# omkhairate/MetalPathtracer

Hardware: AMD Instinct MI355X
Metric: Mrays/s at 1920x1080x256spp on scene.xml (higher is better)
Workload: dtype f32; 1 GPU; scene.xml 1920x1080 x 256 spp per step, depth 8 (181 steps timed); prims=4971, bvh_nodes=2289, bvh_builder=device, rng=philox4x32-10 (pixel,sample,bounce), pipeline=wave-local wavefront, reference-order walk, parallelism=8x8-tile interleave over 1 rank(s), rays=161154900585

## Files before the change

metalpathtracer_amd/csrc/mpt_device.h:

```cpp
#pragma once
#include <hip/hip_runtime.h>
#include <stdint.h>

#include "mpt_lean_entry.h"
#include "mpt_lean_tiles.h"
#include "mpt_lds_cfg.h"

#define MPT_WAVE 64
#define MPT_NSHARD 16
#define MPT_NGROUP 8
#define MPT_NONE 0xFFFFFFFFu

struct F3 {
    float x, y, z;
};
__device__ __forceinline__ F3 f3(float x, float y, float z) { return F3{x, y, z}; }
__device__ __forceinline__ F3 operator+(F3 a, F3 b) { return F3{a.x + b.x, a.y + b.y, a.z + b.z}; }
__device__ __forceinline__ F3 operator-(F3 a, F3 b) { return F3{a.x - b.x, a.y - b.y, a.z - b.z}; }
__device__ __forceinline__ F3 operator*(F3 a, float s) { return F3{a.x * s, a.y * s, a.z * s}; }
__device__ __forceinline__ F3 operator*(float s, F3 a) { return F3{s * a.x, s * a.y, s * a.z}; }
__device__ __forceinline__ F3 operator-(F3 a) { return F3{-a.x, -a.y, -a.z}; }
__device__ __forceinline__ float dot3(F3 a, F3 b) { return a.x * b.x + a.y * b.y + a.z * b.z; }
__device__ __forceinline__ F3 cross3(F3 a, F3 b) {
    return F3{a.y * b.z - a.z * b.y, a.z * b.x - a.x * b.z, a.x * b.y - a.y * b.x};
// ... 139 lines not shown
typedef const __attribute__((address_space(3))) uint32_t* LdsWords;

struct SceneDev {
    const float4* nodes;
    const float4* prims;
    const float4* mats;
    uint32_t n_nodes;
    uint32_t n_lds_nodes;
    uint32_t n_lds_prims;
    uint32_t n_lds_mats;
    uint32_t n_prims;
    uint32_t n_mats;
    uint32_t lds_prim_off;
    uint32_t lds_mat_off;
};
__device__ __forceinline__ int prim_type(float4 p0) { return __float_as_int(p0.w) & 1; }
__device__ __forceinline__ uint32_t prim_ref_leaf(float4 p0) { return (uint32_t)__float_as_int(p0.w) >> 1; }

#ifdef MPT_CLOCK_STAMP
__device__ unsigned long long g_clock[2];
#define MPT_CLOCK_BEGIN() const unsigned long long clk_t0_ = __builtin_amdgcn_s_memtime(), clk_r0_ = __builtin_amdgcn_s_memrealtime()
#define MPT_CLOCK_END()                                                                    \
    do {                                                                                   \
        if ((threadIdx.x & 63u) == 0) {                                                    \
            atomicAdd(&g_clock[0], __builtin_amdgcn_s_memtime() - clk_t0_);                \
            atomicAdd(&g_clock[1], __builtin_amdgcn_s_memrealtime() - clk_r0_);            \
        }                                                                                  \
    } while (0)
#else
#define MPT_CLOCK_BEGIN() do { } while (0)
#define MPT_CLOCK_END() do { } while (0)
#endif

__device__ __forceinline__ bool first_active_lane() {
    const uint32_t me = __builtin_amdgcn_mbcnt_hi(~0u, __builtin_amdgcn_mbcnt_lo(~0u, 0u));
    return me == (uint32_t)__builtin_amdgcn_readfirstlane((int)me);
}

__device__ __forceinline__ uint32_t wave_max_u32(uint32_t v) {
#pragma unroll
    for (int off = 32; off > 0; off >>= 1) {
        const uint32_t other = (uint32_t)__shfl_xor((int)v, off);
        v = other > v ? other : v;
    }
    return v;
}

struct WorkCount {
    uint32_t node_visits, aabb_hits, prim_tests;
    uint32_t node_iters, prim_iters, outer_iters;
#ifdef MPT_DEBUG_WAVE_TIMES
    unsigned long long t_box, t_leaf;
    uint32_t wait_leaf, wait_done;
#endif
#ifdef MPT_OT_TIMES
    unsigned long long ot_node_cycles, ot_leaf_cycles, ot_node_trips, ot_leaf_trips, ot_rounds;
    unsigned long long ot_node_lanes, ot_leaf_lanes;
    unsigned long long ot_lds_nodes, ot_glb_nodes, ot_lds_prims, ot_glb_prims;
    unsigned long long ot_pops, ot_pop_iters, ot_pop_calls, ot_pop_wave_iters;
#endif
};
#ifdef MPT_DEBUG_WAVE_TIMES
#define MPT_TIC(var) unsigned long long var = __builtin_amdgcn_s_memtime()
#define MPT_TOC(acc, var)                                          \
    do {                                                           \
        unsigned long long now_ = __builtin_amdgcn_s_memtime();    \
        (acc) += now_ - (var);                                     \
        (var) = now_;                                              \
    } while (0)
#else
#define MPT_TIC(var) do { } while (0)
#define MPT_TOC(acc, var) do { } while (0)
#endif
struct BoxLoopIdle {
#ifdef MPT_DEBUG_WAVE_TIMES
    uint32_t my_trips = 0, round_trips = 0;
    __device__ __forceinline__ void trip(bool searching) {
        my_trips += searching ? 1u : 0u;
        round_trips++;
    }
    template <bool COUNT>
    __device__ __forceinline__ void book(bool holds_leaf, WorkCount& wc) const {
        if (!COUNT) return;
        if (holds_leaf) wc.wait_leaf += round_trips - my_trips;
        else wc.wait_done += round_trips - my_trips;
    }
#else
    __device__ __forceinline__ void trip(bool) {}
    template <bool COUNT>
    __device__ __forceinline__ void book(bool, WorkCount&) const {}
#endif
};

struct Prim3 {
    float4 p0, p1, p2;
};
typedef const __attribute__((address_space(3))) char* LdsBytes;
__device__ __forceinline__ uint32_t mul_u24(uint32_t a, uint32_t b) { return (uint32_t)__umul24(a, b); }
__device__ __forceinline__ void sphere_cam_terms(F3 o, float4 p0, float4& p1, float4& p2) {
    const F3 oc = o - f3(p0.x, p0.y, p0.z);
    const float radius = p1.x;
    p1.z = dot3(oc, oc) - radius * radius;
    p2.x = oc.x;
    p2.y = oc.y;
    p2.z = oc.z;
}
template <bool LEAN = false, bool PRIMARY = false>
__device__ __forceinline__ Prim3 load_prim(const SceneDev& sc, LdsNodes lds, uint32_t i, F3 o = F3{0.0f, 0.0f, 0.0f}) {
    Prim3 r;
    if (LEAN) {
        const uint32_t off = mul_u24(i, 48u);
        if (i < sc.n_lds_prims) {
            const LdsNodes q = (LdsNodes)((LdsBytes)lds + (sc.lds_prim_off * 16u + off));
            const v4f a = q[0], b = q[1], c = q[2];
            r.p0 = make_float4(a.x, a.y, a.z, a.w);
            r.p1 = make_float4(b.x, b.y, b.z, b.w);
            r.p2 = make_float4(c.x, c.y, c.z, c.w);
        } else {
            const float4* q = (const float4*)((const char*)sc.prims + off);
            r.p0 = q[0];
            r.p1 = q[1];
            r.p2 = q[2];
            if (PRIMARY && prim_type(r.p0) == 0) sphere_cam_terms(o, r.p0, r.p1, r.p2);
        }
        return r;
    }
    if (i < sc.n_lds_prims) {
        const LdsNodes q = lds + sc.lds_prim_off + 3u * i;
        const v4f a = q[0], b = q[1], c = q[2];
        r.p0 = make_float4(a.x, a.y, a.z, a.w);
        r.p1 = make_float4(b.x, b.y, b.z, b.w);
        r.p2 = make_float4(c.x, c.y, c.z, c.w);
    } else {
        r.p0 = sc.prims[3 * i];
        r.p1 = sc.prims[3 * i + 1];
        r.p2 = sc.prims[3 * i + 2];
    }
    return r;
}

// ... 38 lines not shown
            const float cc = cam_terms ? p1.z : dot3(oc, oc) - radius * radius;
            const float disc = b * b - a * cc;
            if (!(b >= 0.0f) && disc > 0.0f) {
                const float sq = sqrtf(disc);
                const float temp = (-b - sq) / a;
                const bool closer = temp < best_t && temp > 0.0001f;
                best_t = closer ? temp : best_t;
                best_prim = closer ? (int)(first + k) : best_prim;
            }
        }
    }
}


#ifndef MPT_LEAF_EARLY
#define MPT_LEAF_EARLY 8u
#endif
#define MPT_NODE_HOLD 0x80000000u
__device__ __forceinline__ bool slab_hit(float4 n0, float4 n1, F3 o, float idx, float idy, float idz, float best_t) {
    float t0 = (n0.x - o.x) * idx, t1 = (n1.x - o.x) * idx;
    float lo = fmaxf(0.0001f, idx < 0.0f ? t1 : t0);
    float hi = fminf(best_t, idx < 0.0f ? t0 : t1);
    t0 = (n0.y - o.y) * idy;
    t1 = (n1.y - o.y) * idy;
    lo = fmaxf(lo, idy < 0.0f ? t1 : t0);
    hi = fminf(hi, idy < 0.0f ? t0 : t1);
    t0 = (n0.z - o.z) * idz;
    t1 = (n1.z - o.z) * idz;
    lo = fmaxf(lo, idz < 0.0f ? t1 : t0);
    hi = fminf(hi, idz < 0.0f ? t0 : t1);
    return hi > lo;
}
static_assert(MPT_LEAN_LEAF_BIT == MPT_NODE_HOLD && MPT_NODE_TAIL < MPT_NODE_HOLD, "mpt_lean_entry.h: the leaf bit and the tail marker");
template <bool COUNT, bool ALL_LDS, bool BUDGETED, bool LEAN = false, bool PRIMARY = false>
__device__ __forceinline__ bool closest_hit_resume(const SceneDev& sc, LdsNodes lds_nodes, F3 o, F3 d, uint32_t& node,
                                                   float& best_t, int& best_prim, uint32_t budget, WorkCount& wc,
                                                   uint32_t min_active = 0u, LdsNodes tail_cfg = nullptr, uint32_t tile_class = 0u) {
    constexpr bool TILES = PRIMARY && LEAN && ALL_LDS;
    const bool tile_skip = TILES && (tile_class & MPT_LEAN_TILES_SKIP) != 0u;
    float idx = 0.0f, idy = 0.0f, idz = 0.0f;
    const uint32_t n_nodes = sc.n_nodes, n_lds = sc.n_lds_nodes;
    uint32_t i = (tile_class & MPT_LEAN_TILES_MASK_BITS) != 0u ? MPT_NODE_TAIL : n_nodes;
    if (!tile_skip) {
    mpt_rcp3(d.x, d.y, d.z, idx, idy, idz);
    i = (d.x != d.x || d.y != d.y || d.z != d.z) ? n_nodes : node;
    uint32_t trips = 0;
    MPT_TIC(tic_);
    for (;;) {
        uint32_t skip = 0;
        unsigned long long search_mask = __ballot(i < n_nodes);
        const uint32_t n_entered0 = (uint32_t)__popcll(search_mask), n_entered = max(n_entered0, 1u);
        BoxLoopIdle idle;
        uint32_t n_searching = n_entered0;
        while (n_searching * MPT_LEAF_EARLY >= n_entered && (!BUDGETED || trips < budget)) {
            const bool searching = LEAN ?__builtin_amdgcn_inverse_ballot_w64(search_mask) : i < n_nodes;
            idle.trip(searching);
            const uint32_t j = LEAN ? i : (i < n_nodes - 1u ? i : n_nodes - 1u);
            float4 n0 = make_float4(0, 0, 0, 0), n1 = n0;
            bool box = false;
            if (searching) {
                if (ALL_LDS || j < n_lds) {
                    const v4f a = lds_nodes[2 * j], b = lds_nodes[2 * j + 1];
                    n0 = make_float4(a.x, a.y, a.z, a.w);
                    n1 = make_float4(b.x, b.y, b.z, b.w);
                } else {
                    n0 = sc.nodes[2 * j];
                    n1 = sc.nodes[2 * j + 1];
                }
                box = slab_hit(n0, n1, o, idx, idy, idz, best_t);
            }
            const uint32_t A = __float_as_uint(n0.w), B = __float_as_uint(n1.w);
            if (COUNT) {
                wc.node_visits += searching ? 1u : 0u;
                wc.aabb_hits += (searching && box) ? 1u : 0u;
                if (first_active_lane()) wc.node_iters++;
            }
            const uint32_t next = box ? A : B;
            i = searching ? next : i;
            skip = searching ? B : skip;
            if (BUDGETED) trips++;
            search_mask = __ballot(i < n_nodes);
            n_searching = (uint32_t)__popcll(search_mask);
        }
        idle.template book<COUNT>((i & MPT_NODE_HOLD) != 0u, wc);
        MPT_TOC(wc.t_box, tic_);
        if ((i & MPT_NODE_HOLD) != 0u) {
            const uint32_t enc = i & ~MPT_NODE_HOLD;
            if (COUNT && first_active_lane()) wc.outer_iters++;
            leaf_test<COUNT, LEAN, PRIMARY>(sc, lds_nodes, enc >> 4, (enc & 15u) + 1u, o, d, best_t, best_prim, wc);
            i = skip;
        }
        MPT_TOC(wc.t_leaf, tic_);
        if (BUDGETED && trips >= budget) break;
        const unsigned long long going = __ballot(i < n_nodes);
        if (going == 0ull) break;
        if (BUDGETED && (uint32_t)__popcll(going) < min_active) break;
    }
    }
    if (LEAN && ALL_LDS) {
        if (i == MPT_NODE_TAIL) {
            const bool d_ok = fmaxf(fmaxf(fabsf(d.x), fabsf(d.y)), fabsf(d.z)) <= MPT_LEAN_ENTRY_DMAX;
            bool hit;
            uint32_t leaf;
            if (PRIMARY) {
                const LdsWords w = (LdsWords)tail_cfg;
                leaf = w[CFG_TAIL_W_LEAF];
                hit = d_ok && w[CFG_TAIL_W_PRIMARY] != 0u;
            } else {
                const v4f tlo = tail_cfg[CFG_TAIL_LO], thi = tail_cfg[CFG_TAIL_HI];
                leaf = __float_as_uint(tlo.w);
                hit = d_ok && tlo.x <= o.x && o.x <= thi.x && tlo.y <= o.y && o.y <= thi.y && tlo.z <= o.z && o.z <= thi.z;
            }
#if !defined(MPT_LEAN_TAIL_NO_SLAB)
            if (__ballot(!hit) != 0ull) {
                if (!hit) {
                    const v4f a = tail_cfg[CFG_TAIL_N0], b = tail_cfg[CFG_TAIL_N1];
                    hit = slab_hit(make_float4(a.x, a.y, a.z, a.w), make_float4(b.x, b.y, b.z, b.w), o, idx, idy, idz, best_t);
                }
            }
#endif
            if (hit) {
                const uint32_t enc = (uint32_t)__builtin_amdgcn_readfirstlane((int)leaf) & ~MPT_NODE_HOLD;
                if (TILES) {
                    uint32_t m = tile_skip ? tile_class & MPT_LEAN_TILES_MASK_BITS : (2u << (enc & 15u)) - 1u;
                    do {
                        const uint32_t s = (uint32_t)__builtin_ctz(m), run = (uint32_t)__builtin_ctz(~(m >> s));
                        leaf_test<COUNT, LEAN, PRIMARY>(sc, lds_nodes, (enc >> 4) + s, run, o, d, best_t, best_prim, wc);
                        m &= ~(((1u << run) - 1u) << s);
                    } while (m != 0u);
                } else {
                    leaf_test<COUNT, LEAN, PRIMARY>(sc, lds_nodes, enc >> 4, (enc & 15u) + 1u, o, d, best_t, best_prim, wc);
                }
            }
        }
    }
    node = i;
    return i >= n_nodes;
}

template <bool COUNT, bool ALL_LDS>
__device__ __forceinline__ void closest_hit(const SceneDev& sc, LdsNodes lds_nodes, F3 o, F3 d,
                                            float& best_t, int& best_prim, WorkCount& wc) {
    uint32_t node = 0;
    best_t = INFINITY;
    best_prim = -1;
    closest_hit_resume<COUNT, ALL_LDS, false>(sc, lds_nodes, o, d, node, best_t, best_prim, 0xFFFFFFFFu, wc);
}

struct HitInfo {
// ... 162 lines not shown
```

metalpathtracer_amd/csrc/mpt_hip.hip:

```cpp
#include <hip/hip_runtime.h>

#include <math.h>
#include <stdint.h>
#include <stdio.h>
#include <string.h>

#include <algorithm>
#include <chrono>
#include <condition_variable>
#include <deque>
#include <mutex>
#include <thread>
#include <map>
#include <memory>
#include <exception>
#include <string>
#include <type_traits>
#include <vector>

#include "mpt.h"
#include "mpt_accel.h"
#include "mpt_scene_layout.h"
#include "mpt_env.h"
#include "mpt_device.h"
// ... 205 lines not shown
    std::unique_ptr<Submitter> sub;
    uint64_t async_jobs = 0;
    uint64_t gate_resident = 0;
    uint64_t gate_timeout = 0;
    uint64_t async_call_us_max = 0;
    hipStream_t stream = nullptr;
    Lane lane[2];
    int next_lane = 0;
    hipEvent_t last_resolved = nullptr;
    hipEvent_t last_traced = nullptr;
    int resolve_wgs_per_cu = 2;
    bool sync_render = false;
    uint32_t launch_seq = 0;
    Lane* last_trace_lane = nullptr;
    int lane_order = 5;
    Event ev_sum_op;
    hipDeviceProp_t prop;
    std::string err;
    std::mutex err_mu;
    bool have_scene = false;
    struct OtPoint {
        uint32_t threads, wgs_per_cu, lds_nodes, lds_prims;
    } ot_pt[2] = {{MPT_OT_THREADS, MPT_OT_WGS_PER_CU, 0, 0}, {MPT_OT6_THREADS, (MPT_OT6_WAVES * 256) / MPT_OT6_THREADS, 0, 0}};
    int ot_occ = 0;
    bool tile_order_forced = false;
    uint32_t ot_stack_depth = 8;
    mpt_build::ScratchPool build_pool;
    DevMem<> spare_block;
    DevMem<> in_block;
    OtBudgets ot_budgets = default_ot_budgets();
    float acc_cull_rel = 9.765625e-4f;
    mpt_uniforms u;
    bool have_uniforms = false;
    uint32_t W = 0, H = 0;
    DevMem<float4> d_accum[2];
    int cur_target = 0;
    DevMem<float4> d_sum_own;
    float4* d_sum = nullptr;
    DevMem<uint32_t> d_tile_xy;
    uint32_t tile_W = 0, tile_H = 0, tile_rank = 0, tile_nranks = 0, tile_count = 0;
    int tile_mode_built = -1;
    int tile_order_mode = 0;
    DevMem<uint32_t> d_pixel_seed;
    float seed_rs[3] = {NAN, NAN, NAN};
    uint32_t seed_W = 0, seed_H = 0;
    int wg_size = 0;
    const void* occ_fun = nullptr;
    size_t occ_lds = 0;
    int occ_per_cu = 0;
    bool time_kernels = true;
    WaveBudgets budgets = default_budgets();
    uint32_t wl_min = 0, wl_div = 32;
    bool wl_lean = true;
    bool lean_tiles = true;
    bool lean_sky_resolve = true;
    LeanCdivCache lean_cdiv;
    DevMem<uint32_t> d_cdiv_bad;
    uint32_t wl_block = MPT_WL_BLOCK;
    int wgs_per_cu = 0;
    size_t lds_budget = 78 * 1024;
    mpt_stats stats = {};
    uint64_t guide_epoch = 1;
    uint64_t tile_class_builds = 0;
    GuideState gd;
    DenoiseState dn;
    DevMem<float4> d_m2;
    AdaptiveTiles ad;
    TemporalState tp;
    SvgfState sv;
    DisplayState dp;
    AoState ao;
    LightState lights;
    DirectState di;
    RestirState rs;
    NeeState nee;
    int32_t light_sampling = MPT_LIGHT_SAMPLING_AREA;
    uint32_t light_candidates = 1u;
    int dp_px = 4;
    bool dp_hist_agg = true;
};

struct TraceKernel {
    const void* fn;
    const char* name;
    int wg_max;
};
enum { TK_PLAIN = 0, TK_CORUN = 1, TK_LEAN = 2, TK_SIX = 4 };
static const struct TraceKernelRow {
    int pipeline;
    bool count, all_lds;
    int variant;
    TraceKernel k;
} g_trace_kernels[] = {
    {MPT_PIPE_WAVEFRONT, true, true, TK_PLAIN, {(const void*)k_step<true, true>, "k_step", 1024}},
    {MPT_PIPE_WAVEFRONT, true, false, TK_PLAIN, {(const void*)k_step<true, false>, "k_step", 1024}},
    {MPT_PIPE_WAVEFRONT, false, true, TK_PLAIN, {(const void*)k_step<false, true>, "k_step", 1024}},
    {MPT_PIPE_WAVEFRONT, false, false, TK_PLAIN, {(const void*)k_step<false, false>, "k_step", 1024}},
    {MPT_PIPE_MEGAKERNEL, true, true, TK_PLAIN, {(const void*)k_megakernel<true, true>, "k_megakernel", 1024}},
    {MPT_PIPE_MEGAKERNEL, true, false, TK_PLAIN, {(const void*)k_megakernel<true, false>, "k_megakernel", 1024}},
    {MPT_PIPE_MEGAKERNEL, false, true, TK_PLAIN, {(const void*)k_megakernel<false, true>, "k_megakernel", 1024}},
    {MPT_PIPE_MEGAKERNEL, false, false, TK_PLAIN, {(const void*)k_megakernel<false, false>, "k_megakernel", 1024}},
    {MPT_PIPE_ORDERED, false, true, TK_SIX, {(const void*)k_ordered<false, true, MPT_OT6_WAVES>, "k_ordered", MPT_OT6_THREADS}},
    {MPT_PIPE_ORDERED, false, false, TK_SIX, {(const void*)k_ordered<false, false, MPT_OT6_WAVES>, "k_ordered", MPT_OT6_THREADS}},
    {MPT_PIPE_ORDERED, true, true, TK_PLAIN, {(const void*)k_ordered<true, true>, "k_ordered", MPT_OT_THREADS}},
    {MPT_PIPE_ORDERED, true, false, TK_PLAIN, {(const void*)k_ordered<true, false>, "k_ordered", MPT_OT_THREADS}},
    {MPT_PIPE_ORDERED, false, true, TK_PLAIN, {(const void*)k_ordered<false, true>, "k_ordered", MPT_OT_THREADS}},
// ... 56 lines not shown
        case MPT_ERR_INVALID_ARG: return "invalid argument";
        case MPT_ERR_NO_DEVICE: return "no HIP device";
        case MPT_ERR_HIP: return "HIP runtime error";
        case MPT_ERR_BAD_SCENE: return "malformed scene arrays";
        case MPT_ERR_NOT_READY: return "scene, uniforms or size not set";
        case MPT_ERR_OVERFLOW: return "ray queue overflow";
    }
    return "unknown status";
}
extern "C" const char* mpt_last_error(const mpt_ctx* ctx) { return ctx ? ctx->err.c_str() : "null context"; }

static int create_impl(int device_ordinal, mpt_ctx** out) {
    if (!out) return MPT_ERR_INVALID_ARG;
    *out = nullptr;
    int n = 0;
    if (hipGetDeviceCount(&n) != hipSuccess || n <= 0) return MPT_ERR_NO_DEVICE;
    if (device_ordinal < 0 || device_ordinal >= n) return MPT_ERR_NO_DEVICE;
    std::unique_ptr<mpt_ctx> ctx(new mpt_ctx());
    ctx->device = device_ordinal;
    if (hipSetDevice(device_ordinal) != hipSuccess) return MPT_ERR_HIP;
    if (hipGetDeviceProperties(&ctx->prop, device_ordinal) != hipSuccess) return MPT_ERR_HIP;
    if (const char* lo = getenv("MPT_LANE_ORDER")) ctx->lane_order = atoi(lo);
    if (const char* rw = getenv("MPT_RESOLVE_WGS")) ctx->resolve_wgs_per_cu = std::max(0, atoi(rw));
    int prio_lo = 0, prio_hi = 0;
    if (hipDeviceGetStreamPriorityRange(&prio_lo, &prio_hi) != hipSuccess) prio_lo = prio_hi = 0;
    for (Lane& L : ctx->lane) {
        const int prio = &L == &ctx->lane[0] ? prio_hi : prio_lo;
        if (((ctx->lane_order & 2) ? L.stream.create(hipStreamCreateWithPriority, hipStreamNonBlocking, prio)
                                   : L.stream.create(hipStreamCreateWithFlags, hipStreamNonBlocking)) != hipSuccess ||
            L.d_desc.alloc(sizeof(PassDesc)) != hipSuccess || hipMemset(L.d_desc.get(), 0, sizeof(PassDesc)) != hipSuccess ||
            L.d_ctr.alloc(MPT_CTR_WORDS * 4) != hipSuccess || hipMemset(L.d_ctr.get(), 0, MPT_CTR_WORDS * 4) != hipSuccess ||
            L.h_done.alloc(64, hipHostMallocMapped) != hipSuccess || L.h_desc.alloc(sizeof(PassDesc)) != hipSuccess ||
            L.ev0.create(hipEventCreate) != hipSuccess || L.ev1.create(hipEventCreate) != hipSuccess ||
            L.ev_resolved.create(hipEventCreate) != hipSuccess || L.ev_traced.create(hipEventCreateWithFlags, hipEventDisableTiming) != hipSuccess)
            return MPT_ERR_HIP;
        memset((void*)L.h_done.get(), 0, 64);
    }
    ctx->stream = ctx->lane[0].stream.get();
    if (ctx->ev_sum_op.create(hipEventCreate) != hipSuccess) return MPT_ERR_HIP;
    const char* e;
    if ((e = getenv("MPT_WG_SIZE"))) ctx->wg_size = atoi(e);
    if ((e = getenv("MPT_WGS_PER_CU"))) ctx->wgs_per_cu = atoi(e);
    if ((e = getenv("MPT_LDS_BYTES"))) ctx->lds_budget = (size_t)atol(e);
    ctx->time_kernels = !((e = getenv("MPT_NO_KERNEL_EVENTS")) && atoi(e));
    if ((e = getenv("MPT_WL_BLOCK")) && atoi(e) >= 64) ctx->wl_block = (uint32_t)atoi(e) & ~63u;
    if ((e = getenv("MPT_DISPLAY_PX")) && (atoi(e) == 1 || atoi(e) == 4)) ctx->dp_px = atoi(e);
    if ((e = getenv("MPT_DISPLAY_HIST"))) ctx->dp_hist_agg = strcmp(e, "plain") != 0;
    if ((e = getenv("MPT_BUDGETS"))) fill_budgets(e, ctx->budgets.b, MPT_WL_LEVELS - 1u);
    if ((e = getenv("MPT_MIN_ACTIVE"))) fill_min_active(e, ctx->budgets.min_active, MPT_WL_LEVELS);
    if ((e = getenv("MPT_LIGHT_BUDGET")) && atoi(e) >= 1) {
        uint32_t b = (uint32_t)atoi(e);
        for (uint32_t k = 0; k + 1 < MPT_WL_LEVELS; ++k) ctx->budgets.b[k] = b > (1u << 28) ? b : std::min<uint64_t>((uint64_t)b << k, MPT_WL_NO_BUDGET);
    }
    if ((e = getenv("MPT_WL_MIN")) && atoi(e) >= 64) ctx->wl_min = (uint32_t)atoi(e) & ~63u;
    if ((e = getenv("MPT_TILE_ORDER"))) {
        ctx->tile_order_mode = atoi(e);
        ctx->tile_order_forced = true;
    }
    if ((e = getenv("MPT_OT_OCC")) && (atoi(e) == 5 || atoi(e) == 6)) ctx->ot_occ = atoi(e);
    if ((e = getenv("MPT_WL_DIV")) && atoi(e) >= 1) ctx->wl_div = (uint32_t)atoi(e);
    if ((e = getenv("MPT_WL_LEAN"))) ctx->wl_lean = atoi(e) != 0;
    if ((e = getenv("MPT_LEAN_TILES"))) ctx->lean_tiles = atoi(e) != 0;
    if ((e = getenv("MPT_LEAN_SKY_RESOLVE"))) ctx->lean_sky_resolve = atoi(e) != 0;
    if ((e = getenv("MPT_OT_STACK")) && atoi(e) >= 2 && atoi(e) <= (int)MPT_OT_PARK) ctx->ot_stack_depth = (uint32_t)atoi(e);
    unsigned ot[MPT_OT_MLEVELS];
    if ((e = getenv("MPT_OT_BUDGETS")))
        for (unsigned k = 0, n = parse_uint_list(e, ot, MPT_OT_MLEVELS); k < n && k + 1 < MPT_OT_MLEVELS; ++k) ctx->ot_budgets.trips[k] = ot[k] < 1 ? 1 : ot[k];
    if ((e = getenv("MPT_OT_MIN_ACTIVE")))
        for (unsigned k = 0, n = parse_uint_list(e, ot, MPT_OT_MLEVELS); k < n; ++k) ctx->ot_budgets.min_active[k] = ot[k] > 64 ? 64 : ot[k];
    if ((e = getenv("MPT_OT_INPLACE")) && atoi(e) >= 1) ctx->ot_budgets.inplace_min = (uint32_t)atoi(e);
    if ((e = getenv("MPT_OT_CULL_REL")) && atof(e) > 0.0) ctx->acc_cull_rel = (float)atof(e);
    if (ctx->wg_size < 64 || ctx->wg_size > 1024 || (ctx->wg_size & 63)) ctx->wg_size = 0;
    if (ctx->lds_budget > 160 * 1024) ctx->lds_budget = 160 * 1024;
    for (const TraceKernelRow& r : g_trace_kernels) hipFuncSetAttribute(r.k.fn, hipFuncAttributeMaxDynamicSharedMemorySize, 160 * 1024);
    hipFuncSetAttribute((const void*)k_trace_rays_ordered, hipFuncAttributeMaxDynamicSharedMemorySize, 160 * 1024);
    hipFuncSetAttribute((const void*)k_trace_rays, hipFuncAttributeMaxDynamicSharedMemorySize, 160 * 1024);
    hipFuncSetAttribute((const void*)k_dn_guide, hipFuncAttributeMaxDynamicSharedMemorySize, 160 * 1024);
    for (const void* k : {(const void*)k_occluded_ref<false>, (const void*)k_occluded_ref<true>, (const void*)k_occluded_own, (const void*)k_ao<MPT_AO_REF>,
                          (const void*)k_ao<MPT_AO_REF_ALL_LDS>, (const void*)k_ao<MPT_AO_OWN>, (const void*)k_direct<MPT_AO_REF>,
                          (const void*)k_direct<MPT_AO_REF_ALL_LDS>, (const void*)k_direct<MPT_AO_OWN>, (const void*)k_nee<MPT_AO_REF>,
                          (const void*)k_nee<MPT_AO_REF_ALL_LDS>, (const void*)k_nee<MPT_AO_OWN>, (const void*)k_direct_cone<MPT_AO_REF>,
                          (const void*)k_direct_cone<MPT_AO_REF_ALL_LDS>, (const void*)k_direct_cone<MPT_AO_OWN>, (const void*)k_nee_cone<MPT_AO_REF>,
                          (const void*)k_nee_cone<MPT_AO_REF_ALL_LDS>, (const void*)k_nee_cone<MPT_AO_OWN>, (const void*)k_nee_adaptive<MPT_AO_REF>,
                          (const void*)k_nee_adaptive<MPT_AO_REF_ALL_LDS>, (const void*)k_nee_adaptive<MPT_AO_OWN>,
                          (const void*)k_nee_adaptive_cone<MPT_AO_REF>, (const void*)k_nee_adaptive_cone<MPT_AO_REF_ALL_LDS>,
                          (const void*)k_nee_adaptive_cone<MPT_AO_OWN>, (const void*)k_restir_initial<MPT_AO_REF>,
                          (const void*)k_restir_initial<MPT_AO_REF_ALL_LDS>, (const void*)k_restir_initial<MPT_AO_OWN>,
                          (const void*)k_restir_merge<MPT_AO_REF, true>, (const void*)k_restir_merge<MPT_AO_REF_ALL_LDS, true>,
                          (const void*)k_restir_merge<MPT_AO_OWN, true>, (const void*)k_restir_merge<MPT_AO_REF, false>,
                          (const void*)k_restir_merge<MPT_AO_REF_ALL_LDS, false>, (const void*)k_restir_merge<MPT_AO_OWN, false>})
        hipFuncSetAttribute(k, hipFuncAttributeMaxDynamicSharedMemorySize, 160 * 1024);
    *out = ctx.release();
    return MPT_OK;
}

extern "C" int mpt_destroy(mpt_ctx* ctx) {
    if (!ctx) return MPT_ERR_INVALID_ARG;
    stop_submit(ctx);
    hipSetDevice(ctx->device);
    for (Lane& L : ctx->lane)
        if (L.stream) hipStreamSynchronize(L.stream.get());
    delete ctx;
    return MPT_OK;
}

static void size_lds_images(mpt_ctx* ctx) {
// ... 444 lines not shown
    return slots_items;
}

static int fill_pass_params(mpt_ctx* ctx, Lane& L, const mpt_render_params* p, uint32_t sample_begin, uint32_t S, int tile_mode,
                            const TileOverride* ovr, PassParams& pp) {
    const uint32_t tiles_x = (ctx->W + 7) / 8;
    pp.scene = scene_dev(ctx);
    for (int i = 0; i < 2; ++i) pp.q[i] = QueueDev{L.q_od[i].get(), L.q_dt[i].get(), L.q_tl[i].get(), L.q_ia[i].get()};
    pp.shard_cap = L.shard_cap;
    pp.desc = L.d_desc.get();
    pp.ctr = L.d_ctr.get();
    pp.slots = L.d_slots.get();
    pp.pixel_seed = ctx->d_pixel_seed.get();
    const mpt_uniforms& u = ctx->u;
    pp.cam = F3{u.cameraPosition[0], u.cameraPosition[1], u.cameraPosition[2]};
    pp.first = F3{u.firstPixelPosition[0], u.firstPixelPosition[1], u.firstPixelPosition[2]};
    pp.vu = F3{u.viewportU[0], u.viewportU[1], u.viewportU[2]};
    pp.vv = F3{u.viewportV[0], u.viewportV[1], u.viewportV[2]};
    pp.W = u.screenSize[0];
    pp.H = u.screenSize[1];
    pp.width = ctx->W;
    pp.height = ctx->H;
    pp.tiles_x = tiles_x;
    pp.S = S;
    pp.s_shift = (S & (S - 1)) == 0 ? (uint32_t)__builtin_ctz(S) : 0xFFu;
    pp.tile_xy = ovr ? ovr->tiles : ctx->d_tile_xy.get();
    pp.sample_begin = sample_begin;
    pp.rank = (uint32_t)p->shard_rank;
    pp.nranks = (uint32_t)p->shard_count;
    {
        const uint64_t tiles = (uint64_t)tiles_x * ((ctx->H + 7) / 8);
        pp.tile_magic = 0u;
        if (!ovr && tile_mode == 0 && tiles_x >= 2u && tiles * tiles_x < (1ull << 32) && getenv("MPT_TILE_TABLE") == nullptr)
            pp.tile_magic = (uint32_t)(((1ull << 32) + tiles_x - 1u) / tiles_x);
    }
    pp.sp.rng_mode = p->rng_mode;
    pp.sp.bsdf_mode = p->bsdf_mode;
    pp.sp.max_depth = p->max_depth;
    pp.sp.seed_lo = p->seed_lo;
    pp.sp.seed_hi = p->seed_hi;
    pp.sp.primitive_count = (uint32_t)std::min<uint64_t>(u.primitiveCount, 0xFFFFFFFFull);
    uint32_t* dev_done = nullptr;
    HIPCHK(hipHostGetDevicePointer((void**)&dev_done, L.h_done.get(), 0));
    pp.host_done = dev_done;
    return MPT_OK;
}

static int select_trace_kernel(mpt_ctx* ctx, Lane& L, const mpt_render_params* p, uint32_t n_local_tiles, const PassParams& pp, PassLaunch& g) {
    const bool count = count_flag(p);
    bool all_lds = ref_all_lds(ctx);
    int variant = TK_PLAIN;
    if (g.pipeline == MPT_PIPE_WAVELOCAL) {
        g.corun = (ctx->lane_order & 4) && !ctx->sync_render && !count;
        const bool lean = ctx->wl_lean &&
                          wl_lean_ok(ctx->n_prims, n_local_tiles, pp.tiles_x, ctx->W, ctx->H, pp.nranks, pp.S, pp.tile_magic, p->rng_mode, p->bsdf_mode, count, &g.lean_args) &&
                          lean_cdiv_ok(ctx->lean_cdiv, pp.W, pp.H, [&](float W, float H, uint32_t* bad) { return lean_cdiv_device_check(ctx, L.stream.get(), W, H, bad); });
        variant = (g.corun ? TK_CORUN : 0) | (lean ? TK_LEAN : 0);
        g.lean_all_lds = lean && all_lds;
    } else if (g.pipeline == MPT_PIPE_ORDERED) {
        g.ot_point = ordered_point(ctx, count);
        all_lds = ctx->ot_pt[g.ot_point].lds_nodes == ctx->n_acc_nodes;
        variant = g.ot_point == 1 ? TK_SIX : TK_PLAIN;
    }
    g.k = trace_kernel(g.pipeline, count, all_lds, variant);
    if (!g.k) return fail(ctx, MPT_ERR_INVALID_ARG, "no trace kernel for this pass (internal)");
    g.wg = g.pipeline != MPT_PIPE_ORDERED && ctx->wg_size > 0 && ctx->wg_size <= g.k->wg_max ? ctx->wg_size : g.k->wg_max;
    return MPT_OK;
}

static int launch_geometry(mpt_ctx* ctx, PassParams& pp, PassLaunch& g) {
    WalkViews v;
    const int vrc = walk_views(ctx, g.pipeline == MPT_PIPE_ORDERED, g.ot_point, (uint32_t)g.wg, v);
    if (vrc) return vrc;
    pp.scene = v.sc;
    g.accel = v.ac;
    g.lds = v.lds;
    int per_cu = 0;
    if (ctx->occ_fun == g.k->fn && ctx->occ_lds == g.lds) {
        per_cu = ctx->occ_per_cu;
    } else {
        HIPCHK(hipOccupancyMaxActiveBlocksPerMultiprocessor(&per_cu, g.k->fn, g.wg, g.lds));
        ctx->occ_fun = g.k->fn;
        ctx->occ_lds = g.lds;
        ctx->occ_per_cu = per_cu;
    }
    if (per_cu < 1) return fail(ctx, MPT_ERR_HIP, "kernel does not fit on a CU");
    if (getenv("MPT_DEBUG_LAUNCH"))
        fprintf(stderr, "[mpt] pipeline %d: %d workgroups of %d per CU, %zu B of LDS each, kernel %s\n", g.pipeline, per_cu, g.wg, g.lds, g.k->name);
    if (ctx->wgs_per_cu > 0 && per_cu > ctx->wgs_per_cu) per_cu = ctx->wgs_per_cu;
    g.grid = ctx->prop.multiProcessorCount * per_cu;
    return MPT_OK;
}

static int order_behind_previous_trace(mpt_ctx* ctx, Lane& L, bool corun) {
    bool need_chain = (ctx->lane_order & 1) != 0;
    if (corun && ctx->last_trace_lane && ctx->last_trace_lane != &L) {
        Lane& O = *ctx->last_trace_lane;
        bool resident = false;
        if (O.announced_id != 0u) {
            const volatile uint32_t* flag = (const volatile uint32_t*)O.h_done.get() + MPT_HOST_RESIDENT;
            const auto t0 = std::chrono::steady_clock::now();
            for (;;) {
                if (*flag == O.announced_id || hipEventQuery(O.ev_traced.get()) == hipSuccess) {
                    resident = true;
                    break;
                }
                if (std::chrono::steady_clock::now() - t0 > std::chrono::milliseconds(200)) break;
// ... 1078 lines not shown
```

metalpathtracer_amd/csrc/mpt_kernels.h:

```cpp
#pragma once
#include <hip/hip_runtime.h>
#include <stdint.h>

#include "mpt_device.h"
#include "mpt_wl_lean.h"
#include "mpt_lean_entry.h"
#include "mpt_lean_tiles.h"

#ifndef MPT_MIN_WAVES
#define MPT_MIN_WAVES 8
#endif

struct QueueDev {
    float4* od;
    float4* dt;
    float4* tl;
    uint2* ia;
};

struct PassDesc {
    uint32_t in_count[MPT_NSHARD];
    uint32_t item_prefix[MPT_NSHARD + 1];
    uint32_t n_items;
    uint32_t regen_base;
// ... 610 lines not shown
                                                                                                  const uint32_t* tile_classes, uint32_t sky_resolve) {
    wavelocal_body<false, ALL_LDS, true>(pp, ring, budgets, wl_block, wl_min, wl_div, lean, tile_classes, sky_resolve);
}
template <bool ALL_LDS>
__global__ __launch_bounds__(MPT_WL_THREADS(ALL_LDS), MPT_WL_WAVES(ALL_LDS)) __attribute__((amdgpu_num_sgpr(MPT_WL_CORUN_SGPRS)))
void k_wavelocal_lean_corun(PassParams pp, WaveRings ring, WaveBudgets budgets, uint32_t wl_block, uint32_t wl_min, uint32_t wl_div, WlLean lean,
                            const uint32_t* tile_classes, uint32_t sky_resolve) {
    wavelocal_body<false, ALL_LDS, true>(pp, ring, budgets, wl_block, wl_min, wl_div, lean, tile_classes, sky_resolve);
}
__global__ __launch_bounds__(64) void k_lean_tile_classes(const float4* nodes, uint32_t n_nodes, const float4* prims, uint32_t n_prims, LeanTileView view,
                                                          uint32_t* out, uint32_t n_words) {
    const uint32_t T = blockIdx.x * blockDim.x + threadIdx.x;
    if (T >= n_words) return;
    const uint32_t ty = T / view.tiles_x, tx = T - ty * view.tiles_x;
    out[T] = ty < view.tiles_y ? lean_tile_class(nodes, n_nodes, prims, n_prims, view, tx, ty) : 0u;
}
struct WaveStepDiag {
    enum Region { SELECT, FETCH, TRACE, SHADE, PUSH, N_REGIONS };
#ifdef MPT_DEBUG_WAVE_TIMES
    unsigned long long t_start, t_exh = 0ull, t_claim = 0ull, steps = 0ull, left = 0ull, blk = 0ull;
    unsigned long long reg[N_REGIONS] = {}, tic_;
    WorkCount wc0;
    __device__ __forceinline__ static uint32_t n_waves() { return gridDim.x * (blockDim.x >> 6); }
    __device__ __forceinline__ static unsigned long long* buffer(const WaveRings& ring) { return (unsigned long long*)(ring.tv() + (size_t)n_waves() * MPT_WL_LEVELS * MPT_WL_RING); }
    __device__ __forceinline__ void start() { t_start = __builtin_amdgcn_s_memrealtime(); }
    __device__ __forceinline__ void tic() { tic_ = __builtin_amdgcn_s_memtime(); }
    __device__ __forceinline__ void toc(Region r) { MPT_TOC(reg[r], tic_); }
    __device__ __forceinline__ void claimed(bool got, uint32_t asked, const uint32_t* cnt) {
        if (got) {
            t_claim = __builtin_amdgcn_s_memrealtime();
            steps = 0ull;
            blk = asked;
        } else {
            t_exh = __builtin_amdgcn_s_memrealtime();
            for (uint32_t q = 0; q < MPT_WL_LEVELS; ++q) left |= (unsigned long long)cnt[q] << (12u * q);
        }
    }
    __device__ __forceinline__ void step(bool exhausted, int level) {
        if (!exhausted) steps += 1ull << (12u * (uint32_t)(level + 1));
    }
    __device__ __forceinline__ void before_walk(const WorkCount& wc) { wc0 = wc; }
    template <bool COUNT>
    __device__ __forceinline__ void after_walk(const WaveRings& ring, int level, const WorkCount& wc, bool done) const {
        if (!COUNT) return;
        unsigned long long* lv = buffer(ring) + 16ull * n_waves() + 8ull * (unsigned)(level + 1);
        if (first_active_lane()) atomicAdd(lv + 0, 1ull);
        if (wc.node_iters != wc0.node_iters) atomicAdd(lv + 1, (unsigned long long)(wc.node_iters - wc0.node_iters));
        if (wc.prim_iters != wc0.prim_iters) atomicAdd(lv + 3, (unsigned long long)(wc.prim_iters - wc0.prim_iters));
        atomicAdd(lv + 2, (unsigned long long)(wc.node_visits - wc0.node_visits));
        atomicAdd(lv + 4, (unsigned long long)(wc.prim_tests - wc0.prim_tests));
        atomicAdd(lv + 5, 1ull);
        if (wc.wait_leaf != wc0.wait_leaf) atomicAdd(lv + 7, (unsigned long long)(wc.wait_leaf - wc0.wait_leaf));
        if (done) atomicAdd(lv + 6, 1ull);
    }
    template <bool COUNT>
    __device__ __forceinline__ void traffic(const WaveRings& ring, uint32_t lane, unsigned long long am, unsigned long long pm, bool keep, bool alive, bool parked,
                                            const PathState& ps) const {
        if (!COUNT || (am | pm) == 0ull) return;
        unsigned long long* rt = buffer(ring) + 16ull * n_waves() + 8ull * 14ull;
        const unsigned long long lit_a = __ballot(alive && ring_has_light(ps)), lit_p = __ballot(parked && ring_has_light(ps));
        if (lane == 0u) {
            if (am != 0ull) {
                atomicAdd(rt + 8 + (keep ? 0 : 1), (unsigned long long)__popcll(am));
                atomicAdd(rt + 8 + (keep ? 2 : 3), (unsigned long long)__popcll(lit_a));
                atomicAdd(rt + 8 + (keep ? 4 : 5), 1ull);
            }
            if (pm != 0ull) {
                atomicAdd(rt + 0, (unsigned long long)__popcll(pm));
                atomicAdd(rt + 1, (unsigned long long)__popcll(lit_p));
                atomicAdd(rt + 2, 1ull);
            }
        }
    }
    __device__ __forceinline__ void finish(const WaveRings& ring, uint32_t lane, uint32_t wave_id, const WorkCount& wc) const {
        if (lane != 0) return;
        unsigned long long* dbg = buffer(ring);
        dbg[8 * wave_id] = t_start;
        dbg[8 * wave_id + 1] = t_exh;
        dbg[8 * wave_id + 2] = __builtin_amdgcn_s_memrealtime();
        dbg[8 * wave_id + 3] = t_claim;
        dbg[8 * wave_id + 4] = steps;
        dbg[8 * wave_id + 5] = left;
        dbg[8 * wave_id + 6] = blk;
        unsigned long long* out = dbg + 8ull * n_waves() + 8ull * wave_id;
        for (int r = 0; r < N_REGIONS; ++r) out[r] = reg[r];
        out[5] = wc.t_box;
        out[6] = wc.t_leaf;
    }
#else
    __device__ __forceinline__ void start() {}
    __device__ __forceinline__ void tic() {}
    __device__ __forceinline__ void toc(Region) {}
    __device__ __forceinline__ void claimed(bool, uint32_t, const uint32_t*) {}
    __device__ __forceinline__ void step(bool, int) {}
    __device__ __forceinline__ void before_walk(const WorkCount&) {}
    template <bool COUNT>
    __device__ __forceinline__ void after_walk(const WaveRings&, int, const WorkCount&, bool) const {}
    template <bool COUNT>
    __device__ __forceinline__ void traffic(const WaveRings&, uint32_t, unsigned long long, unsigned long long, bool, bool, bool, const PathState&) const {}
    __device__ __forceinline__ void finish(const WaveRings&, uint32_t, uint32_t, const WorkCount&) const {}
#endif
};
template <bool ALL_LDS>
__device__ __forceinline__ void cfg_stage_lean(float4* blk, const PassParams& pp) {
    const float4 none = make_float4(0.0f, 0.0f, 0.0f, 0.0f);
    const bool tree = pp.scene.n_nodes != 0u;
    const LeanEntry e = lean_entry_terms(tree ? pp.scene.nodes[0] : none, tree ? pp.scene.nodes[1] : none, pp.scene.n_nodes, pp.cam.x, pp.cam.y, pp.cam.z);
    uint32_t entry = e.entry, entry_primary = e.entry_primary;
    if (ALL_LDS) {
        const LeanTail t = lean_tail_terms(pp.scene.nodes, pp.scene.n_nodes, pp.cam.x, pp.cam.y, pp.cam.z);
        float4* const tail = blk + CFG_F4_TAIL;
        tail[CFG_TAIL_LO] = make_float4(t.tlo[0], t.tlo[1], t.tlo[2], __uint_as_float(t.leaf));
        tail[CFG_TAIL_HI] = make_float4(t.thi[0], t.thi[1], t.thi[2], __uint_as_float(t.tail_primary));
        float4 t0 = make_float4(0.0f, 0.0f, 0.0f, 0.0f), t1 = t0;
        if (t.node != 0u) {
            t0 = pp.scene.nodes[2u * t.node];
            t1 = pp.scene.nodes[2u * t.node + 1u];
        }
        t1.w = __uint_as_float(t.node);
        tail[CFG_TAIL_N0] = t0;
        tail[CFG_TAIL_N1] = t1;
        if (t.node != 0u && entry == t.node) entry = MPT_NODE_TAIL;
        if (t.node != 0u && entry_primary == t.node) entry_primary = MPT_NODE_TAIL;
    }
    blk[CFG_F4_ENTRY_LO] = make_float4(e.ilo[0], e.ilo[1], e.ilo[2], __uint_as_float(entry));
    blk[CFG_F4_ENTRY_HI] = make_float4(e.ihi[0], e.ihi[1], e.ihi[2], __uint_as_float(entry_primary));
}
template <bool COUNT, bool ALL_LDS, bool LEAN>
__device__ __forceinline__ void wavelocal_body(const PassParams& pp, const WaveRings& ring, const WaveBudgets& budgets, uint32_t wl_block, uint32_t wl_min,
                                               uint32_t wl_div, const WlLean& lean, const uint32_t* tile_classes, uint32_t sky_resolve) {
    static_assert(!(LEAN && COUNT), "the lean body does not count");
    constexpr bool TILES = LEAN && ALL_LDS;
    extern __shared__ float4 lds_nodes_raw[];
    const uint32_t cfg_off = mpt_lds_cfg_off_f4(pp.scene.lds_mat_off);
    float4* const blk_raw = lds_nodes_raw + cfg_off;
    if (threadIdx.x == 0) {
        announce_resident(pp);
        cfg_stage_common(blk_raw, pp, LEAN ? cdiv_recip(pp.W) : 0.0f, LEAN ? cdiv_recip(pp.H) : 0.0f, wl_block, wl_min, wl_div);
        uint32_t* w = (uint32_t*)(blk_raw + CFG_F4_WORDS);
        static_assert(MPT_WL_LEVELS <= CFG_MAX_LEVELS, "configuration block: a budget word per ring");
        for (uint32_t k = 0; k < MPT_WL_LEVELS; ++k) {
            w[CFG_W_BUDGET + k] = budgets.b[k];
            w[CFG_W_MIN_ACTIVE + k] = budgets.min_active[k];
        }
        if (LEAN) {
            w[CFG_W_S_MUL] = lean.s_mul;
            w[CFG_W_S_SHIFT] = lean.s_shift;
        }
        if (TILES) {
            w[CFG_W_CLASSES_LO] = (uint32_t)(uintptr_t)tile_classes;
            w[CFG_W_CLASSES_HI] = (uint32_t)((uint64_t)(uintptr_t)tile_classes >> 32);
            static_assert(MPT_WL_LEVELS < CFG_MAX_LEVELS, "configuration block: CFG_W_SKY_RESOLVE lies in the last ring's minimum");
            w[CFG_W_SKY_RESOLVE] = tile_classes != nullptr ? sky_resolve : 0u;
        }
        if (LEAN) cfg_stage_lean<ALL_LDS>(blk_raw, pp);
    }
    if (LEAN) stage_nodes_lean(pp.scene, lds_nodes_raw, pp.cam);
    else stage_nodes(pp.scene, lds_nodes_raw);
    if (LEAN && ALL_LDS) {
        const uint32_t tail_node = __float_as_uint(blk_raw[CFG_F4_TAIL + CFG_TAIL_N1].w);
        if (tail_node != 0u) {
            uint32_t* links = (uint32_t*)lds_nodes_raw;
            for (uint32_t k = threadIdx.x; k < pp.scene.n_lds_nodes * 2u; k += blockDim.x)
                if (links[4u * k + 3u] == tail_node) links[4u * k + 3u] = MPT_NODE_TAIL;
        }
        __syncthreads();
    }
    MPT_CLOCK_BEGIN();
    const LdsNodes lds_nodes = (LdsNodes)lds_nodes_raw;
    const LdsNodes blk = lds_nodes + cfg_off;
    const LdsWords lds_cfg_u32 = (LdsWords)(blk + CFG_F4_WORDS);
    const uint32_t lane = threadIdx.x & 63u;
    const uint32_t wave_id = blockIdx.x * (blockDim.x >> 6) + (threadIdx.x >> 6);
    const uint32_t wbase = wave_id * (MPT_WL_LEVELS * MPT_WL_RING);
    const uint32_t M = MPT_WL_RING - 1u;
    uint32_t cnt[MPT_WL_LEVELS];
#pragma unroll
    for (uint32_t k = 0; k < MPT_WL_LEVELS; ++k) cnt[k] = 0;
    uint32_t cur = 0, end = 0;
    uint32_t grp = blockIdx.x & (MPT_NGROUP - 1u);
    uint32_t seen = 0;
    bool exhausted = false;
    uint32_t tile_cached = 0xFFFFFFFFu, tile_xy_cached = 0u;
    uint32_t tile_class_cached = 0u;
    float uvx_cached = 0.0f, uvy_cached = 0.0f;
// ... 66 lines not shown
                    }
                }
                if (TILES) {
                } else if (LEAN) {
                    const uint32_t T = tl * pp.nranks + pp.rank, ty = (T * lean.tile_mul) >> MPT_WL_LEAN_TILE_SHIFT;
                    tile_xy_cached = (T - ty * pp.tiles_x) | (ty << 16);
                } else {
                    tile_xy_cached = (uint32_t)__builtin_amdgcn_readfirstlane((int)pp.tile_xy[tl]);
                }
            }
            PathState np;
            np.path = pchunk * 64u + lane;
            uint32_t tile_xy = tile_xy_cached;
            if (TILES) {
                const uint32_t T = tl * pp.nranks + pp.rank, ty = (T * lean.tile_mul) >> MPT_WL_LEAN_TILE_SHIFT;
                tile_xy = (T - ty * pp.tiles_x) | (ty << 16);
            }
            const uint32_t px = (tile_xy & 0xFFFFu) * 8u + (lane & 7u), py = (tile_xy >> 16) * 8u + (lane >> 3);
            if (TILES && (tile_class_cached & MPT_WL_TILE_ELIDED) != 0u) {
                const uint32_t left = (end - cur) >> 6, more = pp.S - 1u - sidx < left ? pp.S - 1u - sidx : left;
                const uint32_t elided = (uint32_t)__popcll(__ballot(px < pp.width && py < pp.height)) * (1u + more);
                cur += more * 64u;
                n_paths += elided;
                n_rays += elided;
                continue;
            }
            const CamView cv = cfg_cam_view(blk);
            if (new_tile) pixel_uv(cv, px, py, uvx_cached, uvy_cached);
            if (px < pp.width && py < pp.height) {
                gen_primary<LEAN>(pp, cv, px, py, uvx_cached, uvy_cached, pp.sample_begin + sidx, np, g);
                valid = true;
            }
            n_paths += (uint32_t)__popcll(__ballot(valid));
            ps = np;
        } else {
            uint32_t my_ring = 0, my_off = 0;
            bool take = false;
            uint32_t assigned = 0;
            const uint32_t slot = wave_rank(~carry), room = 64u - (uint32_t)__popcll(carry);
            const bool empty = !kept;
#pragma unroll
            for (int k = (int)MPT_WL_LEVELS - 1; k >= 0; --k) {
                const bool use = (level == (int)MPT_WL_LEVELS) || (level == k);
                uint32_t tk = use ? cnt[k] : 0u;
                tk = tk < room - assigned ? tk : room - assigned;
                if (empty && slot >= assigned && slot < assigned + tk) {
                    take = true;
                    my_ring = (uint32_t)k;
                    my_off = cnt[k] - tk + (slot - assigned);
                }
                cnt[k] -= tk;
                assigned += tk;
            }
            if (level < (int)MPT_WL_LEVELS) {
                budget = (uint32_t)__builtin_amdgcn_readfirstlane((int)lds_cfg_u32[CFG_W_BUDGET + level]);
                min_active = (uint32_t)__builtin_amdgcn_readfirstlane((int)lds_cfg_u32[CFG_W_MIN_ACTIVE + level]);
            }
            if (level == (int)MPT_WL_LEVELS && assigned >= 12u) min_active = assigned / 3u;
            if (take) {
                const uint32_t at = wbase + my_ring * MPT_WL_RING + my_off;
                uint4 tv = make_uint4(0u, 0u, 0u, 0u);
                if (my_ring > 0u) tv = ring.tv()[at];
                ring_pop_hit(ring, at, ps, hit_t, hit_prim);
                need_shade = my_ring == 0u;
                if (my_ring > 0u) {
                    node = tv.x;
                    best_t = __uint_as_float(tv.y);
                    best_prim = (int)tv.z;
                } else {
                    fresh = true;
                }
                valid = true;
            }
            if (kept) {
                need_shade = true;
                fresh = true;
                valid = true;
            }
        }
        if (need_shade) {
            uint32_t px, py, sidx;
            path_to_pixel<LEAN>(pp, ps.path, px, py, sidx, lean.tile_mul, lds_cfg_u32);
            g.pixel = LEAN ? mul_u24(py, pp.width) + px : py * pp.width + px;
            g.sample = pp.sample_begin + sidx;
            g.lit_seed = 0;
            if (!LEAN && pp.sp.rng_mode == 0) g.lit_seed = pcg_hash(pcg_hash(pp.pixel_seed[g.pixel]));
            if (!shade_bounce<LEAN>(pp.scene, lds_nodes, pp.sp, g, ps, hit_t, hit_prim)) {
                store_slot(pp.slots, ps.path, clamp01(ps.L.x), clamp01(ps.L.y), clamp01(ps.L.z), clamp01(ps.La));
                valid = false;
            }
        }
        if (LEAN && fresh) {
            const bool d_ok = fmaxf(fmaxf(fabsf(ps.d.x), fabsf(ps.d.y)), fabsf(ps.d.z)) <= MPT_LEAN_ENTRY_DMAX;
            if (level < 0) {
                const uint32_t entry_primary = ((LdsWords)(blk + CFG_F4_ENTRY_HI))[CFG_W_OF_F4];
                node = d_ok ? entry_primary : 0u;
            } else {
                const v4f elo = blk[CFG_F4_ENTRY_LO], ehi = blk[CFG_F4_ENTRY_HI];
                const bool in = elo.x <= ps.o.x && ps.o.x <= ehi.x && elo.y <= ps.o.y && ps.o.y <= ehi.y && elo.z <= ps.o.z && ps.o.z <= ehi.z;
                node = in && d_ok ? __float_as_uint(elo.w) : 0u;
            }
        }
        const bool budgeted = level >= 0 && (level < (int)MPT_WL_LEVELS || min_active != 0u) &&
                              ((level < (int)MPT_WL_LEVELS - 1 && budget < MPT_WL_NO_BUDGET) || min_active != 0u);
        const int park_ring = level + 1 < (int)MPT_WL_LEVELS ? level + 1 : (int)MPT_WL_LEVELS - 1;
        bool alive = false, parked = false;
        diag.toc(WaveStepDiag::FETCH);
// ... 298 lines not shown
```

metalpathtracer_amd/csrc/mpt_lds_cfg.h:

```cpp
#pragma once
#include <stdint.h>

enum : uint32_t {
    CFG_F4_CAM = 0u,
    CFG_F4_FIRST = 1u,
    CFG_F4_VU = 2u,
    CFG_F4_VV = 3u,
    CFG_F4_WORDS = 4u,
    CFG_F4_ENTRY_LO = 10u,
    CFG_F4_ENTRY_HI = 11u,
    CFG_F4_TAIL = 12u,
    CFG_F4_END = 16u,
    CFG_MAX_LEVELS = 8u,
    CFG_W_BUDGET = 0u,
    CFG_W_MIN_ACTIVE = 8u,
    CFG_W_INPLACE_MIN = 15u,
    CFG_W_SKY_RESOLVE = 15u,
    CFG_W_CLAIM_BLOCK = 16u,
    CFG_W_CLAIM_MIN = 17u,
    CFG_W_CLAIM_DIV = 18u,
    CFG_W_RANK_TILES = 19u,
    CFG_W_S_MUL = 20u,
    CFG_W_S_SHIFT = 21u,
    CFG_W_CLASSES_LO = 22u,
    CFG_W_CLASSES_HI = 23u,
    CFG_N_WORDS = 24u,
    CFG_W_OF_F4 = 3u,
    CFG_TAIL_LO = 0u,
    CFG_TAIL_HI = 1u,
    CFG_TAIL_N0 = 2u,
    CFG_TAIL_N1 = 3u,
    CFG_TAIL_W_LEAF = 4u * CFG_TAIL_LO + CFG_W_OF_F4,
    CFG_TAIL_W_PRIMARY = 4u * CFG_TAIL_HI + CFG_W_OF_F4,
};
static_assert(CFG_W_BUDGET + CFG_MAX_LEVELS <= CFG_W_MIN_ACTIVE && CFG_W_MIN_ACTIVE + CFG_MAX_LEVELS - 1u <= CFG_W_INPLACE_MIN,
              "configuration block: the per-level words overlap (the last minimum shares its word with k_ordered's threshold: MPT_OT_MLEVELS < 8)");
static_assert(4u * CFG_F4_WORDS + CFG_N_WORDS <= 4u * CFG_F4_ENTRY_LO, "configuration block: the word area runs into the entry terms");
static_assert(CFG_F4_ENTRY_HI + 1u <= CFG_F4_TAIL && CFG_F4_TAIL + CFG_TAIL_N1 + 1u <= CFG_F4_END, "configuration block: the lean slots overlap");
```

Measured before the change: 74440 Mrays/s.

## Unroll lean budgeted box loop in pairs and hardwire ring budgets as constants

In the lean budgeted traversal, the box loop now runs two node steps per exit check and tests against a precomputed active-lane threshold, so the ballot-count check runs half as often. For the two-level lean ring, the per-level budget and min-active values become compile-time constants instead of LDS reads with readfirstlane. The lean path is now disabled when budget environment knobs are set. Debug counters for low-occupancy trips and a test-only ring-control option are added. The paired steps can let a wave run one extra trip past the early-leaf threshold or the budget.

```diff
diff --git a/metalpathtracer_amd/csrc/mpt_device.h b/metalpathtracer_amd/csrc/mpt_device.h
--- a/metalpathtracer_amd/csrc/mpt_device.h
+++ b/metalpathtracer_amd/csrc/mpt_device.h
@@ -215,6 +215,7 @@
 #ifdef MPT_DEBUG_WAVE_TIMES
     unsigned long long t_box, t_leaf;
     uint32_t wait_leaf, wait_done;
+    uint32_t low_trips[3];
 #endif
 #ifdef MPT_OT_TIMES
     unsigned long long ot_node_cycles, ot_leaf_cycles, ot_node_trips, ot_leaf_trips, ot_rounds;
@@ -248,7 +249,13 @@
         if (holds_leaf) wc.wait_leaf += round_trips - my_trips;
         else wc.wait_done += round_trips - my_trips;
     }
+    __device__ __forceinline__ static void low(uint32_t n_searching, WorkCount& wc) {
+        wc.low_trips[0] += n_searching < 8u ? 1u : 0u;
+        wc.low_trips[1] += n_searching < 16u ? 1u : 0u;
+        wc.low_trips[2] += n_searching < 24u ? 1u : 0u;
+    }
 #else
+    __device__ __forceinline__ static void low(uint32_t, WorkCount&) {}
     __device__ __forceinline__ void trip(bool) {}
     template <bool COUNT>
     __device__ __forceinline__ void book(bool, WorkCount&) const {}
@@ -393,7 +400,12 @@
         const uint32_t n_entered0 = (uint32_t)__popcll(search_mask), n_entered = max(n_entered0, 1u);
         BoxLoopIdle idle;
         uint32_t n_searching = n_entered0;
-        while (n_searching * MPT_LEAF_EARLY >= n_entered && (!BUDGETED || trips < budget)) {
+        constexpr bool PAIRS = LEAN && BUDGETED;
+        constexpr int TRIPS_PER_CHECK = PAIRS ? 2 : 1;
+        const uint32_t need = PAIRS ? max((n_entered0 + MPT_LEAF_EARLY - 1u) / MPT_LEAF_EARLY, 1u) : 0u;
+        while ((PAIRS ? n_searching >= need : n_searching * MPT_LEAF_EARLY >= n_entered) && (!BUDGETED || trips < budget)) {
+#pragma unroll
+          for (int rep = 0; rep < TRIPS_PER_CHECK; ++rep) {
             const bool searching = LEAN ?__builtin_amdgcn_inverse_ballot_w64(search_mask) : i < n_nodes;
             idle.trip(searching);
             const uint32_t j = LEAN ? i : (i < n_nodes - 1u ? i : n_nodes - 1u);
@@ -414,13 +426,17 @@
             if (COUNT) {
                 wc.node_visits += searching ? 1u : 0u;
                 wc.aabb_hits += (searching && box) ? 1u : 0u;
-                if (first_active_lane()) wc.node_iters++;
+                if (first_active_lane()) {
+                    wc.node_iters++;
+                    BoxLoopIdle::low(n_searching, wc);
+                }
             }
             const uint32_t next = box ? A : B;
             i = searching ? next : i;
             skip = searching ? B : skip;
             if (BUDGETED) trips++;
             search_mask = __ballot(i < n_nodes);
+          }
             n_searching = (uint32_t)__popcll(search_mask);
         }
         idle.template book<COUNT>((i & MPT_NODE_HOLD) != 0u, wc);
@@ -435,7 +451,12 @@
         if (BUDGETED && trips >= budget) break;
         const unsigned long long going = __ballot(i < n_nodes);
         if (going == 0ull) break;
-        if (BUDGETED && (uint32_t)__popcll(going) < min_active) break;
+        if (BUDGETED && (uint32_t)__popcll(going) < min_active) {
+#if defined(MPT_LEAN_RING_CONTROL)
+            if (LEAN && budget < 0x7FFFFFFFu && i < n_nodes) i = n_nodes;
+#endif
+            break;
+        }
     }
     }
     if (LEAN && ALL_LDS) {
diff --git a/metalpathtracer_amd/csrc/mpt_hip.hip b/metalpathtracer_amd/csrc/mpt_hip.hip
--- a/metalpathtracer_amd/csrc/mpt_hip.hip
+++ b/metalpathtracer_amd/csrc/mpt_hip.hip
@@ -281,6 +281,7 @@
     WaveBudgets budgets = default_budgets();
     uint32_t wl_min = 0, wl_div = 32;
     bool wl_lean = true;
+    bool ring_knobs_set = false;
     bool lean_tiles = true;
     bool lean_sky_resolve = true;
     LeanCdivCache lean_cdiv;
@@ -443,6 +444,9 @@
         uint32_t b = (uint32_t)atoi(e);
         for (uint32_t k = 0; k + 1 < MPT_WL_LEVELS; ++k) ctx->budgets.b[k] = b > (1u << 28) ? b : std::min<uint64_t>((uint64_t)b << k, MPT_WL_NO_BUDGET);
     }
+#if !defined(MPT_LEAN_RING_TESTING)
+    ctx->ring_knobs_set = getenv("MPT_BUDGETS") || getenv("MPT_MIN_ACTIVE") || getenv("MPT_LIGHT_BUDGET");
+#endif
     if ((e = getenv("MPT_WL_MIN")) && atoi(e) >= 64) ctx->wl_min = (uint32_t)atoi(e) & ~63u;
     if ((e = getenv("MPT_TILE_ORDER"))) {
         ctx->tile_order_mode = atoi(e);
@@ -993,7 +997,7 @@
     int variant = TK_PLAIN;
     if (g.pipeline == MPT_PIPE_WAVELOCAL) {
         g.corun = (ctx->lane_order & 4) && !ctx->sync_render && !count;
-        const bool lean = ctx->wl_lean &&
+        const bool lean = ctx->wl_lean && !ctx->ring_knobs_set &&
                           wl_lean_ok(ctx->n_prims, n_local_tiles, pp.tiles_x, ctx->W, ctx->H, pp.nranks, pp.S, pp.tile_magic, p->rng_mode, p->bsdf_mode, count, &g.lean_args) &&
                           lean_cdiv_ok(ctx->lean_cdiv, pp.W, pp.H, [&](float W, float H, uint32_t* bad) { return lean_cdiv_device_check(ctx, L.stream.get(), W, H, bad); });
         variant = (g.corun ? TK_CORUN : 0) | (lean ? TK_LEAN : 0);
diff --git a/metalpathtracer_amd/csrc/mpt_kernels.h b/metalpathtracer_amd/csrc/mpt_kernels.h
--- a/metalpathtracer_amd/csrc/mpt_kernels.h
+++ b/metalpathtracer_amd/csrc/mpt_kernels.h
@@ -686,6 +686,12 @@
         atomicAdd(lv + 5, 1ull);
         if (wc.wait_leaf != wc0.wait_leaf) atomicAdd(lv + 7, (unsigned long long)(wc.wait_leaf - wc0.wait_leaf));
         if (done) atomicAdd(lv + 6, 1ull);
+        unsigned long long* lo = lv + 8ull * 8ull;
+        for (int q = 0; q < 3; ++q) {
+            const uint32_t n = wc.low_trips[q] - wc0.low_trips[q];
+            if (n != 0u) atomicAdd(lo + q, (unsigned long long)n);
+            if (__ballot(n != 0u) != 0ull && first_active_lane()) atomicAdd(lo + 3 + q, 1ull);
+        }
     }
     template <bool COUNT>
     __device__ __forceinline__ void traffic(const WaveRings& ring, uint32_t lane, unsigned long long am, unsigned long long pm, bool keep, bool alive, bool parked,
@@ -765,6 +771,11 @@
                                                uint32_t wl_div, const WlLean& lean, const uint32_t* tile_classes, uint32_t sky_resolve) {
     static_assert(!(LEAN && COUNT), "the lean body does not count");
     constexpr bool TILES = LEAN && ALL_LDS;
+#if defined(MPT_LEAN_RING_TESTING)
+    constexpr bool RING_CONSTS = false;
+#else
+    constexpr bool RING_CONSTS = LEAN && MPT_WL_LEVELS == 2u;
+#endif
     extern __shared__ float4 lds_nodes_raw[];
     const uint32_t cfg_off = mpt_lds_cfg_off_f4(pp.scene.lds_mat_off);
     float4* const blk_raw = lds_nodes_raw + cfg_off;
@@ -937,7 +948,12 @@
                 cnt[k] -= tk;
                 assigned += tk;
             }
-            if (level < (int)MPT_WL_LEVELS) {
+            if (RING_CONSTS) {
+                if (level < (int)MPT_WL_LEVELS) {
+                    budget = level == 0 ? MPT_LEAN_RING0_BUDGET : MPT_WL_NO_BUDGET;
+                    min_active = level == 0 ? MPT_LEAN_RING0_N0 : MPT_LEAN_RING1_N;
+                }
+            } else if (level < (int)MPT_WL_LEVELS) {
                 budget = (uint32_t)__builtin_amdgcn_readfirstlane((int)lds_cfg_u32[CFG_W_BUDGET + level]);
                 min_active = (uint32_t)__builtin_amdgcn_readfirstlane((int)lds_cfg_u32[CFG_W_MIN_ACTIVE + level]);
             }
diff --git a/metalpathtracer_amd/csrc/mpt_lds_cfg.h b/metalpathtracer_amd/csrc/mpt_lds_cfg.h
--- a/metalpathtracer_amd/csrc/mpt_lds_cfg.h
+++ b/metalpathtracer_amd/csrc/mpt_lds_cfg.h
@@ -33,6 +33,16 @@
     CFG_TAIL_W_LEAF = 4u * CFG_TAIL_LO + CFG_W_OF_F4,
     CFG_TAIL_W_PRIMARY = 4u * CFG_TAIL_HI + CFG_W_OF_F4,
 };
+#ifndef MPT_LEAN_RING0_BUDGET
+#define MPT_LEAN_RING0_BUDGET 8u
+#endif
+#ifndef MPT_LEAN_RING0_N0
+#define MPT_LEAN_RING0_N0 8u
+#endif
+#define MPT_LEAN_RING1_N 24u
+#if defined(MPT_LEAN_RING_CONTROL) && !defined(MPT_LEAN_RING_TESTING)
+#error "MPT_LEAN_RING_CONTROL makes a parked ray forget what it had found: test builds only (-DMPT_LEAN_RING_TESTING)"
+#endif
 static_assert(CFG_W_BUDGET + CFG_MAX_LEVELS <= CFG_W_MIN_ACTIVE && CFG_W_MIN_ACTIVE + CFG_MAX_LEVELS - 1u <= CFG_W_INPLACE_MIN,
               "configuration block: the per-level words overlap (the last minimum shares its word with k_ordered's threshold: MPT_OT_MLEVELS < 8)");
 static_assert(4u * CFG_F4_WORDS + CFG_N_WORDS <= 4u * CFG_F4_ENTRY_LO, "configuration block: the word area runs into the entry terms");
```

Measured after the change: 75980 Mrays/s (median of 6 runs). 2.1% higher.
